# ictnlp/StreamSpeech

Measured on NVIDIA H100. Metric: audio-seconds/sec (RTF^-1) Fr-En simul S2ST @chunk=320ms, higher is better.
Workload: dtype f32

## Files before the change

### streamspeech_b200/csrc/engine.h

```cpp
#pragma once
#include <cuda_runtime.h>

#include <map>
#include <tuple>
#include <utility>
#include <string>
#include <vector>

#include "../../include/streamspeech_b200.h"
#include "kernels.h"
#include "kernels_persist.h"
#include "kernels_multistream.h"

namespace ss {

struct HostTensor {
  std::vector<float> data;
  std::vector<int64_t> shape;
  int64_t numel() const {
    int64_t n = 1;
    for (auto s : shape) n *= s;
    return n;
  }
};
// ... 53 lines not shown
};

}

struct ss_engine {
  int device = 0;
  ss_config cfg{};
  std::string err;
  bool finalized = false;
  int attn_chunk = 8, conv_chunk = 8;
  int umma_vocoder = 0;
  int umma_linear = 0;
  int unit_grouped = 1;
  int umma_min_rows = 128;
  int umma_min_channels = 16;
  ss::Umma2Cache* umma2_cache = nullptr;
  int vocoder_streams = 1;
  cudaStream_t aux_stream[2] = {nullptr, nullptr};
  cudaEvent_t fork_event = nullptr, join_event[2] = {nullptr, nullptr};
  int vocoder_graph = 0;
  int graph_pdl = 0;
  cudaStream_t capture_stream = nullptr;
  std::map<std::tuple<int, uintptr_t, int, int, int>, std::pair<cudaGraphExec_t, int>> voc_graphs;
  float* persist_ffn_scratch = nullptr;
  float* cl_blobs = nullptr;
  int cluster_cooperative = 1;
  long long cl_steps = 0;
  int persistent_encoder_cluster = 0;
  int persistent_ffn_fused = 1;
  int fbank_tma = 1;
  int persistent_encoder = 1;
  std::map<std::string, ss::HostTensor> host;
  std::vector<void*> dev_allocs;

  ss::Linear sub_conv[2];
  ss::Linear enc_linear;
  std::vector<ss::ConformerLayerW> enc;
  int Tpos = 0;
  ss::Linear ctc_head[2];
  ss::Linear ctc_pair;
  unsigned* ctc_ticket = nullptr;
  float* mt_emb = nullptr;
  float* mt_pos = nullptr;
  int mt_pos_rows = 0;
  std::vector<ss::DecLayerW> mt;
  ss::LNorm mt_ln;
// ... 86 lines not shown
```

### streamspeech_b200/csrc/engine_run.cu

```cuda
#include <algorithm>
#include <cmath>
#include <cstring>
#include <stdexcept>
#include <tuple>

#include "engine.h"

using namespace ss;

namespace {

inline cudaStream_t S(void* s) { return (cudaStream_t)s; }

int check_launch(ss_engine* h, const char* where) {
  cudaError_t e = cudaGetLastError();
  if (e != cudaSuccess) return h->fail(SS_ERR_CUDA, std::string(where) + ": " + cudaGetErrorString(e));
  return SS_OK;
}

thread_local int g_umma_linear = 0;
thread_local int g_umma_conv = 0;
thread_local int g_umma_min_rows = 128;
thread_local int g_umma_min_channels = 16;
thread_local Umma2Cache* g_umma2_cache = nullptr;
// ... 65 lines not shown
  Epilogue e;
  e.out = out; e.ldo = ldo; e.act = act;
  return e;
}
Epilogue ep_residual(float* inout, int ldo, float alpha = 1.0f) {
  Epilogue e;
  e.out = inout; e.ldo = ldo; e.alpha = alpha; e.residual = inout; e.res_scale = 1.0f;
  return e;
}

int report_async_error(ss_engine* h, unsigned flag, const char* where) {
  if (!flag) return SS_OK;
  cudaDeviceSynchronize();
  if (h->persist_bar) cudaMemset(h->persist_bar, 0, 64 * sizeof(unsigned));
  h->persist_bar_target = 0;
  return h->fail(SS_ERR_CUDA, std::string(where) + ": a grid barrier of a persistent kernel timed out; the results of the calls since the "
                                                   "last check are invalid (barrier re-armed)");
}

void clear_graphs(ss_engine* h) {
  cudaDeviceSynchronize();
  for (auto& kv : h->voc_graphs) cudaGraphExecDestroy(kv.second.first);
  h->voc_graphs.clear();
}

bool ws_begin(ss_engine* h, size_t bytes) {
  h->ws.reset();
  return h->ws.ensure(bytes);
}

struct DecScratch {
  float *y, *q, *kv, *attn, *hid, *qkv;
};

void dec_layer(const DecLayerW& L, float* x, int n, int dim, int ffn, int heads, bool causal, int self_kv_len_limit,
               const int* self_kv_len_dev, float* cache_k, float* cache_v, int past, const float* cross_kv, int Tk,
               const int* cross_len_dev, DecScratch& s, cudaStream_t st, int group_R = 0, const int* group_len_dev = nullptr) {
  const float scale = 0.125f;
  if (group_R > 1 && !cache_k && causal && n % group_R == 0) {
    const int S = n / group_R;
    ln_linear(x, dim * group_R, S, L.self_ln, L.qkv, ep_out(s.qkv, 3 * dim), s.y, st);
    grouped_causal_attention(s.qkv, 3 * dim, s.qkv + dim, 3 * dim, s.qkv + 2 * dim, 3 * dim, s.attn, dim, S, group_R, heads, scale, group_len_dev, st);
  } else if (cache_k) {
    ln_qkv_routed(x, dim, n, L.self_ln, L.qkv, dim, s.q, dim, cache_k + (size_t)past * dim, dim, cache_v + (size_t)past * dim, dim, s.y, st);
    mha_attention(s.q, dim, cache_k, dim, cache_v, dim, s.attn, dim, 1, n, past + n, heads, scale, 1, past, self_kv_len_dev, st);
  } else {
    ln_linear(x, dim, n, L.self_ln, L.qkv, ep_out(s.qkv, 3 * dim), s.y, st);
    mha_attention(s.qkv, 3 * dim, s.qkv + dim, 3 * dim, s.qkv + 2 * dim, 3 * dim, s.attn, dim, 1, n, n, heads, scale,
                  causal ? 1 : 0, 0, self_kv_len_dev, st);
  }
  (void)self_kv_len_limit;
// ... 774 lines not shown
  const int nrb = c.voc_n_rb;
  size_t total = ((size_t)N * c.voc_in_dim + (size_t)(2 + 4 * nrb) * maxbuf + (size_t)N * h->hop + 8192) * sizeof(float) + 64 * 256;
  if (!ws_begin(h, total)) return h->fail(SS_ERR_CUDA, "workspace allocation failed");
  float* frames = h->ws.f32((size_t)N * c.voc_in_dim);
  float* bufX = h->ws.f32(maxbuf);
  float* bufY = h->ws.f32(maxbuf);
  std::vector<float*> rbA(nrb), rbB(nrb), rbT(nrb), rbO(nrb);
  bool ok = frames && bufX && bufY;
  for (int j = 0; j < nrb; ++j) {
    rbA[j] = h->ws.f32(maxbuf); rbB[j] = h->ws.f32(maxbuf); rbT[j] = h->ws.f32(maxbuf); rbO[j] = h->ws.f32(maxbuf);
    ok = ok && rbA[j] && rbB[j] && rbT[j] && rbO[j];
  }
  float* wav = h->ws.f32((size_t)N * h->hop);
  if (!ok || !wav) return h->fail(SS_ERR_CUDA, "workspace too small");
  const bool fan_out = h->vocoder_streams && nrb == 3 && (g_umma_conv == 0 || g_umma_conv >= 12);
  if (fan_out && !h->fork_event) {
    bool made = cudaEventCreateWithFlags(&h->fork_event, cudaEventDisableTiming) == cudaSuccess;
    for (int i = 0; i < 2 && made; ++i)
      made = cudaStreamCreateWithFlags(&h->aux_stream[i], cudaStreamNonBlocking) == cudaSuccess &&
             cudaEventCreateWithFlags(&h->join_event[i], cudaEventDisableTiming) == cudaSuccess;
    if (!made) return h->fail(SS_ERR_CUDA, "cannot create the vocoder's auxiliary streams");
  }
  expand_frames(h->voc_unit_emb, h->voc_cumsum, h->voc_U, f_lo, N, c.voc_embedding_dim, frames, st);
  auto generator_body = [&](cudaStream_t st) {
  {
    ConvA a;
    a.x = frames; a.B = 1; a.L_in = N; a.L_rows = N; a.C_in = c.voc_in_dim; a.ldx = c.voc_in_dim; a.ksize = 7; a.pad_left = 3;
    Epilogue e = ep_out(bufX, c.voc_init_channels);
    e.bias = h->conv_pre.lin.b;
    conv_gemm(a, h->conv_pre.lin.w, c.voc_init_channels, e, st);
  }
  int L = N, ch = c.voc_init_channels;
  for (int i = 0; i < c.voc_n_ups; ++i) {
    const UpsampleW& U = h->ups[i];
    const int Lout = L * U.u;
    const bool fan_up = fan_out && U.u > 1;
    if (fan_up) {
      cudaEventRecord(h->fork_event, st);
      for (int q = 0; q < 2; ++q) cudaStreamWaitEvent(h->aux_stream[q], h->fork_event, 0);
    }
    for (int phi = 0; phi < U.u; ++phi) {
      int J = U.phase_J[phi], q0 = U.phase_q0[phi];
      int qmax = (Lout - 1 - phi + U.pad) / U.u;
      int nrows = qmax - q0 + 1;
      if (nrows <= 0) continue;
      const int lane = fan_up ? phi % 3 : 0;
// ... 111 lines not shown
  else if (n == "umma_linear") h->umma_linear = value;
  else if (n == "umma_min_rows") h->umma_min_rows = value;
  else if (n == "umma_min_channels") h->umma_min_channels = value;
  else if (n == "umma2_cache_clear") {
    umma2_cache_clear(h->umma2_cache);
    clear_graphs(h);
  }
  else if (n == "umma2_split_below") { g_umma2_split_below = value; clear_graphs(h); }
  else if (n == "umma2_min_units") { g_umma2_min_units = value; clear_graphs(h); }
  else if (n == "umma2_debug") {
    if (value && !g_umma2_dbg) {
      if (cudaMalloc(&g_umma2_dbg, 16 * sizeof(unsigned long long)) != cudaSuccess) return h->fail(SS_ERR_CUDA, "cudaMalloc failed");
      cudaMemset(g_umma2_dbg, 0, 16 * sizeof(unsigned long long));
    }
    if (!value && g_umma2_dbg) {
      cudaDeviceSynchronize();
      cudaFree(g_umma2_dbg);
      g_umma2_dbg = nullptr;
    }
  }
  else if (n == "prefer_shared") g_prefer_shared = value;
  else if (n == "unit_grouped") h->unit_grouped = value;
  else if (n == "vocoder_graph") h->vocoder_graph = value;
  else if (n == "graph_pdl") h->graph_pdl = value;
  else if (n == "fbank_tma") h->fbank_tma = value;
  else if (n == "umma2_fused_reduce") g_umma2_fused_reduce = value;
  else if (n == "persistent_encoder") h->persistent_encoder = value;
  else if (n == "persistent_ffn_fused") h->persistent_ffn_fused = value;
  else if (n == "cluster_cooperative") h->cluster_cooperative = value;
  else if (n == "persistent_encoder_cluster") {
    if (value && !h->cl_blobs) {
      if (!h->persist_layers || !h->persist_bar) return h->fail(SS_ERR_STATE, "persistent_encoder_cluster needs a finalized engine");
      const size_t n_f = encoder_layers_cluster_blob_floats(h->cfg.enc_layers);
      if (h->cfg.enc_dim != 256 || h->cfg.enc_ffn != 2048) return h->fail(SS_ERR_INVALID, "persistent_encoder_cluster: encoder must be 256 / 2048");
      if (cudaMalloc(&h->cl_blobs, n_f * sizeof(float)) != cudaSuccess) return h->fail(SS_ERR_CUDA, "cudaMalloc failed");
      h->dev_allocs.push_back(h->cl_blobs);
      encoder_layers_cluster_pack(h->persist_layers, h->cfg.enc_layers, h->cfg.dw_kernel, h->cl_blobs, 0);
      if (cudaDeviceSynchronize() != cudaSuccess) return h->fail(SS_ERR_CUDA, "packing the cluster weight blobs failed");
    }
    h->persistent_encoder_cluster = value;
  }
  else if (n == "vocoder_streams") h->vocoder_streams = value;
  else if (n == "persistent_mt") h->persistent_mt = value;
  else if (n == "persistent_mt_prefix") h->persistent_mt_prefix = value;
  else if (n == "persistent_mt_v2") h->persistent_mt_v2 = value;
  else if (n == "persistent_prefetch") h->persistent_prefetch = value;
// ... 142 lines not shown
```

### streamspeech_b200/csrc/kernels.h

```cpp
#pragma once
#include <cuda_runtime.h>
#include <stdint.h>

namespace ss {

extern unsigned long long g_launches;
extern int g_prefer_shared;
extern thread_local int g_pdl_off;

enum Act : int { ACT_NONE = 0, ACT_RELU = 1, ACT_SILU = 2, ACT_TANH = 3 };

struct ConvA {
  const float* x = nullptr;
  int B = 1;
  int L_in = 0;
  int L_rows = 0;
  int C_in = 0;
  int ldx = 0;
  int ksize = 1;
  int stride = 1;
  int dil = 1;
  int pad_left = 0;
  int chunk = 0;
  float pre_lrelu = 1.0f;
// ... 20 lines not shown
  const float* ln_beta = nullptr;
  int split_n = 0;
  float* out2 = nullptr;
  float* out3 = nullptr;
  int ldo2 = 0, ldo3 = 0;
};

void gemm_conv(const ConvA& a, const float* W, int N, const Epilogue& ep, cudaStream_t st);

float* splitk_workspace(size_t bytes);
unsigned* splitk_counters(int n_tiles);
void set_splitk_slot(int slot);
void splitk_epilogue(const float* ws, int splits, int M, int N, int L_rows, const Epilogue& ep, cudaStream_t st);

struct Umma2Cache;
extern int g_umma2_split_below, g_umma2_min_units;
extern int g_umma2_fused_reduce;
extern unsigned long long* g_umma2_dbg;
Umma2Cache* umma2_cache_create();
void umma2_cache_clear(Umma2Cache* c);
void umma2_cache_destroy(Umma2Cache* c);
bool umma2_supported(const ConvA& a, int N, const Epilogue& ep);
void umma2_conv(Umma2Cache* cache, const ConvA& a, const float* W, int N, const Epilogue& ep, int pieces, cudaStream_t st);

bool skinny_gemm_supported(int M, int N, int K, const Epilogue& ep);
void skinny_gemm(const float* A, int lda, const float* W, int M, int N, int K, const Epilogue& ep, cudaStream_t st);

void layer_norm(const float* x, int ldx, float* y, int ldy, const float* gamma, const float* beta, int rows, int C,
                cudaStream_t st);

void fbank_cmvn(const float* samples, int64_t n_samples, int f0, int nf, const float* mel_bank ,
                const float* window , const float* cmvn_mean, const float* cmvn_inv_std_or_null,
                const float* cmvn_std, float* out , cudaStream_t st);

void fbank_cmvn_tma(const float* samples, int f0, int nf, const float* melT, const float* window, const float* cmvn_mean, const float* cmvn_std,
                    float* out, cudaStream_t st);

void relpos_attention(const float* q, int ldq, const float* k, int ldk, const float* v, int ldv, const float* pos, int Tpos,
                      const float* bias_u, const float* bias_v, float* out, int B, int nQ, int q_offset, int T, int H, int D,
                      int chunk , const int* lengths_dev, cudaStream_t st);

void mha_attention(const float* q, int ldq, const float* k, int ldk, const float* v, int ldv, float* out, int ldo, int B,
                   int Tq, int Tk, int H, float scale, int causal, int causal_offset, const int* kv_len_dev,
                   cudaStream_t st);

void grouped_causal_attention(const float* q, int ldq, const float* k, int ldk, const float* v, int ldv, float* out, int ldo, int S, int R,
// ... 27 lines not shown
```

### streamspeech_b200/csrc/kernels_persist.cu

```cuda
#include <cooperative_groups.h>

#include "common.cuh"
#include "kernels.h"
#include "kernels_persist.h"

namespace cg = cooperative_groups;

namespace ss {
namespace {

constexpr int PW = 8;
constexpr int PT = PW * 32;
constexpr int PMR = 16;
constexpr int PHD = 64;
constexpr int PD = 256;

__device__ __forceinline__ unsigned long long globaltimer_ns() {
  unsigned long long t;
  asm volatile("mov.u64 %0, %globaltimer;" : "=l"(t));
  return t;
}

__device__ __forceinline__ float4 ldw(const float* p) {
  float4 r;
  asm volatile("ld.global.nc.L1::no_allocate.v4.f32 {%0, %1, %2, %3}, [%4];" : "=f"(r.x), "=f"(r.y), "=f"(r.z), "=f"(r.w) : "l"(p));
  return r;
}

__device__ __forceinline__ void grid_barrier(unsigned* ctr, unsigned& target) {
  __syncthreads();
  target += gridDim.x;
  if (threadIdx.x == 0) {
    asm volatile("red.release.gpu.global.add.u32 [%0], 1;" ::"l"(ctr) : "memory");
    unsigned v, spins = 0;
    do {
      asm volatile("ld.relaxed.gpu.global.u32 %0, [%1];" : "=r"(v) : "l"(ctr) : "memory");
    } while ((int)(v - target) < 0 && ++spins < (1u << 20));
    if ((int)(v - target) < 0) atomicExch(ctr + SS_BAR_ERR_WORD, 1u);
    asm volatile("fence.acq_rel.gpu;" ::: "memory");
  }
  __syncthreads();
}

__device__ __forceinline__ void prefetch_l2(const float* p, int n_floats) {
  const int lines = n_floats >> 5;
  for (int i = blockIdx.x * PT + threadIdx.x; i < lines; i += gridDim.x * PT)
    asm volatile("prefetch.global.L2 [%0];" ::"l"(p + (size_t)i * 32));
}

__device__ __forceinline__ void prefetch_layer(const PersistLayer& L, int D, int FFN) {
  prefetch_l2(L.ffn1_w1, D * FFN);
  prefetch_l2(L.ffn1_w2, D * FFN);
  prefetch_l2(L.wqkv, 3 * D * D);
  prefetch_l2(L.wo, D * D);
  prefetch_l2(L.pw1, 2 * D * D);
  prefetch_l2(L.pw2, D * D);
  prefetch_l2(L.ffn2_w1, D * FFN);
  prefetch_l2(L.ffn2_w2, D * FFN);
}

struct GemmEpi {
  const float* bias = nullptr;
  int act = ACT_NONE;
  float alpha = 1.f;
// ... 671 lines not shown
```

### streamspeech_b200/csrc/kernels_persist.h

```cpp
#pragma once
#include <cuda_runtime.h>
#include <stdint.h>

namespace ss {

#define SS_BAR_ERR_WORD 32

struct PersistLayer {
  const float *ffn1_g, *ffn1_b, *ffn1_w1, *ffn1_b1, *ffn1_w2, *ffn1_b2;
  const float *attn_g, *attn_b, *wqkv, *bqkv, *wo, *bo, *pos_u, *pos_v, *pos_proj;
  const float *conv_g, *conv_b, *pw1, *pw1_b, *dw_w, *bn_scale, *bn_shift, *pw2, *pw2_b;
  const float *ffn2_g, *ffn2_b, *ffn2_w1, *ffn2_b1, *ffn2_w2, *ffn2_b2;
  const float *fin_g, *fin_b;
  const float *ffn1_w2t, *ffn2_w2t;
};

bool encoder_layers_persistent_supported(int nA, int D, int FFN, int H, int T, int dw_k);
int encoder_layers_persistent(const PersistLayer* layers_dev, int n_layers, float* x, float* hid, float* qb, float* att, float* dw, float* kc,
                              float* vc, float* gc, int nA, int a0, int T, int D, int FFN, int H, int Tpos, int chunk, int conv_chunk, int dw_k,
                              unsigned long long* timestamps_or_null, unsigned* barrier_counter_dev_or_null,
                              unsigned* barrier_target_host, int prefetch ,
                              float* ffn_scratch_or_null , cudaStream_t st);

size_t encoder_layers_cluster_blob_floats(int n_layers);
void encoder_layers_cluster_pack(const PersistLayer* layers_dev, int n_layers, int dw_k, float* blobs_dev, cudaStream_t st);
bool encoder_layers_cluster_supported(int nA, int D, int FFN, int H, int T, int dw_k);
int encoder_layers_cluster(const PersistLayer* layers_dev, const float* blobs_dev, int n_layers, float* x, float* kc, float* vc, float* gc, int nA,
                           int a0, int T, int Tpos, int chunk, int conv_chunk, int dw_k, unsigned* bar_ctr, unsigned* bar_target_host,
                           unsigned long long* ts_or_null, const float* const* pos_proj_host , int cooperative ,
// ... 29 lines not shown
```

### streamspeech_b200/csrc/kernels_persist_mt.cu

```cuda
#include "common.cuh"
#include "kernels.h"
#include "kernels_persist.h"

namespace ss {
namespace {

constexpr int MW = 8;
constexpr int MTT = MW * 32;
constexpr int MHD = 64;

__device__ __forceinline__ float4 ldw(const float* p) {
  float4 r;
  asm volatile("ld.global.nc.L1::no_allocate.v4.f32 {%0, %1, %2, %3}, [%4];" : "=f"(r.x), "=f"(r.y), "=f"(r.z), "=f"(r.w) : "l"(p));
  return r;
}

__device__ __forceinline__ void grid_barrier(unsigned* ctr, unsigned& target) {
  __syncthreads();
  target += gridDim.x;
  if (threadIdx.x == 0) {
    asm volatile("red.release.gpu.global.add.u32 [%0], 1;" ::"l"(ctr) : "memory");
    unsigned v, spins = 0;
    do {
      asm volatile("ld.relaxed.gpu.global.u32 %0, [%1];" : "=r"(v) : "l"(ctr) : "memory");
    } while ((int)(v - target) < 0 && ++spins < (1u << 20));
    if ((int)(v - target) < 0) atomicExch(ctr + SS_BAR_ERR_WORD, 1u);
    asm volatile("fence.acq_rel.gpu;" ::: "memory");
  }
  __syncthreads();
}

struct MtSmem {
  float x[512];
  float v[2048];
  float S[1024];
  float qh[MHD];
  float pv[16][MHD];
  float red[MW];
  float rbest[MW];
  int ridx[MW];
  int tok;
};

__device__ __forceinline__ float block_reduce_sum(MtSmem& sm, float v) {
  const int lane = threadIdx.x & 31, w = threadIdx.x >> 5;
  v = warp_sum(v);
  __syncthreads();
  if (lane == 0) sm.red[w] = v;
  __syncthreads();
  float t = sm.red[0];
#pragma unroll
  for (int i = 1; i < MW; ++i) t += sm.red[i];
// ... 713 lines not shown
```

### streamspeech_b200/csrc/kernels_persist_mtp.cu

```cuda
#include "common.cuh"
#include "kernels.h"
#include "kernels_persist.h"

namespace ss {
namespace {

constexpr int QW = 8;
constexpr int QT = QW * 32;
constexpr int QRB = 16;
constexpr int QMAXM = 64;
constexpr int QD = 512;
constexpr int QFFN = 2048;
constexpr int QHD = 64;
constexpr int QMAXT = 1024;

__device__ __forceinline__ float4 ldw(const float* p) {
  float4 r;
  asm volatile("ld.global.nc.L1::no_allocate.v4.f32 {%0, %1, %2, %3}, [%4];" : "=f"(r.x), "=f"(r.y), "=f"(r.z), "=f"(r.w) : "l"(p));
  return r;
}

__device__ __forceinline__ void grid_barrier(unsigned* ctr, unsigned& target) {
  __syncthreads();
  target += gridDim.x;
  if (threadIdx.x == 0) {
    asm volatile("red.release.gpu.global.add.u32 [%0], 1;" ::"l"(ctr) : "memory");
    unsigned v, spins = 0;
    do {
      asm volatile("ld.relaxed.gpu.global.u32 %0, [%1];" : "=r"(v) : "l"(ctr) : "memory");
    } while ((int)(v - target) < 0 && ++spins < (1u << 20));
    if ((int)(v - target) < 0) atomicExch(ctr + SS_BAR_ERR_WORD, 1u);
    asm volatile("fence.acq_rel.gpu;" ::: "memory");
  }
  __syncthreads();
}

struct QSmem {
  float part[QW][4][QRB];
  float qs[QW][QHD];
};

__device__ __forceinline__ void stage_ln512(float* As, const float* x, int M, int Mpad, const float* __restrict__ g, const float* __restrict__ b,
                                            const int64_t* src_tok, const float* __restrict__ emb, const float* __restrict__ pos, int pad,
                                            float emb_scale, float* xg) {
  const int lane = threadIdx.x & 31, warp = threadIdx.x >> 5;
  float gv[16], bv[16];
#pragma unroll
  for (int i = 0; i < 16; ++i) {
    gv[i] = __ldg(g + lane + (i << 5));
    bv[i] = __ldg(b + lane + (i << 5));
  }
  for (int m0 = warp; m0 < Mpad; m0 += 2 * QW) {
    float v[2][16];
#pragma unroll
    for (int u = 0; u < 2; ++u) {
      const int m = m0 + u * QW;
      if (m < M) {
// ... 342 lines not shown
```

### streamspeech_b200/csrc/kernels_umma2.cu

```cuda
#include <cuda_bf16.h>

#include <algorithm>
#include <map>
#include <tuple>
#include <vector>

#include "common.cuh"
#include "kernels.h"

namespace ss {

struct Umma2Cache {
  std::map<std::tuple<const float*, int, int, int, int, int, int>, unsigned char*> packed;
  std::vector<void*> allocs;
};

namespace {

constexpr int U2_BM = 128;
constexpr int U2_CONVERTERS = 256;
constexpr int U2_THREADS = 288;
constexpr int U2_MAX_UNITS = 6;
constexpr int U2_MAX_SB = 4;
constexpr int U2_MAX_HALO = 64;

__device__ __forceinline__ uint32_t smem_u32(const void* p) { return (uint32_t)__cvta_generic_to_shared(p); }

__device__ __forceinline__ float u2_act(float x, int act) {
  switch (act) {
    case ACT_RELU: return x > 0.f ? x : 0.f;
    case ACT_SILU: return x / (1.0f + expf(-x));
// ... 454 lines not shown
  for (void* p : c->allocs) cudaFree(p);
  c->allocs.clear();
  c->packed.clear();
}

void umma2_cache_destroy(Umma2Cache* c) {
  if (!c) return;
  umma2_cache_clear(c);
  delete c;
}

bool umma2_supported(const ConvA& a, int N, const Epilogue& ep) {
  if (a.B != 1 || a.stride != 1 || a.chunk != 0 || a.lengths != nullptr) return false;
  if (a.t_offset != 0 || a.x_row0 != 0 || a.x_rows != 0) return false;
  if ((a.C_in & 15) != 0 || (a.ldx & 3) != 0 || a.C_in > a.ldx) return false;
  if ((reinterpret_cast<uintptr_t>(a.x) & 15) != 0) return false;
  if ((a.ksize - 1) * a.dil > U2_MAX_HALO || a.ksize < 1 || a.dil < 1) return false;
  if (N < 16 || (ep.glu && (N & 1))) return false;
  if (ep.ln_gamma != nullptr || ep.split_n > 0) return false;
  if (ep.out_L > 0 && a.L_rows <= 0) return false;
  return true;
}

void umma2_conv(Umma2Cache* cache, const ConvA& a, const float* W, int N, const Epilogue& ep, int pieces, cudaStream_t st) {
  ++g_launches;
  const int M = a.L_rows;
  if (M <= 0) return;
  const int NP = pieces >= 3 ? 3 : 2;
  const int BN = u2_bn(N);
  const int CK = (a.C_in % 32 == 0) ? 32 : 16;
  const int n_chunks = a.C_in / CK;
  const int n_tiles = (N + BN - 1) / BN;
  const int k = a.ksize;
  auto key = std::make_tuple(W, N, a.C_in, k, BN, NP, CK);
  unsigned char* wp = nullptr;
  auto it = cache->packed.find(key);
  if (it == cache->packed.end()) {
    const size_t bytes = (size_t)n_tiles * n_chunks * k * NP * BN * CK * 2;
    if (cudaMalloc((void**)&wp, bytes) != cudaSuccess) {
      cudaGetLastError();
      --g_launches;
      gemm_conv(a, W, N, ep, st);
      return;
    }
    cache->allocs.push_back(wp);
    cache->packed[key] = wp;
    const int64_t total = (int64_t)n_tiles * n_chunks * k * (CK >> 3) * BN;
    const int blocks = (int)((total + 255) / 256);
    if (NP == 3)
      umma2_pack_kernel<3><<<blocks, 256, 0, st>>>(W, N, a.C_in, k, BN, CK, n_tiles, wp);
    else
      umma2_pack_kernel<2><<<blocks, 256, 0, st>>>(W, N, a.C_in, k, BN, CK, n_tiles, wp);
  } else {
    wp = it->second;
  }
  U2Params p;
  p.a = a;
  p.ep = ep;
  p.wp = wp;
  p.M = M;
  p.N = N;
  p.CK = CK;
  p.ksize = k;
  p.dil = a.dil;
  p.rs = U2_BM + (k - 1) * a.dil;
  p.rs_pad = ((p.rs + 7) & ~7) + 4;
  p.units_total = n_chunks * k;
  const int m_tiles = (M + U2_BM - 1) / U2_BM;
  const long base = (long)m_tiles * n_tiles;
  const int min_units = std::max(1, g_umma2_min_units);
  int splits = 1;
  if (base < g_umma2_split_below && p.units_total >= 2 * min_units) {
    const long sms = std::max(1, current_device_sms());
    splits = (int)std::min<long>((sms + base - 1) / base, p.units_total / min_units);
    while (splits > 1 && (size_t)splits * M * N * sizeof(float) > (32u << 20)) --splits;
  }
  int ups = (p.units_total + splits - 1) / splits;
  splits = (p.units_total + ups - 1) / ups;
// ... 12 lines not shown
  const size_t a_bytes = (size_t)2 * NP * (CK >> 3) * p.rs_pad * 16;
  const size_t b_unit = (size_t)NP * BN * CK * 2;
  p.SB = (((a_bytes + 127) & ~(size_t)127) + 4 * b_unit <= 110 * 1024) ? 4 : 3;
  const size_t smem = std::max<size_t>(((a_bytes + 127) & ~(size_t)127) + p.SB * b_unit, (size_t)U2_BM * (BN + 8) * sizeof(float)) + 256;
  dim3 grid(n_tiles, m_tiles, splits);
  if (NP == 3) {
    switch (BN) {
      case 128: u2_launch<128, 3>(p, grid, smem, st); break;
      case 64: u2_launch<64, 3>(p, grid, smem, st); break;
      case 32: u2_launch<32, 3>(p, grid, smem, st); break;
      default: u2_launch<16, 3>(p, grid, smem, st); break;
    }
  } else {
    switch (BN) {
      case 128: u2_launch<128, 2>(p, grid, smem, st); break;
      case 64: u2_launch<64, 2>(p, grid, smem, st); break;
      case 32: u2_launch<32, 2>(p, grid, smem, st); break;
      default: u2_launch<16, 2>(p, grid, smem, st); break;
    }
  }
  if (splits > 1 && p.tile_ctr == nullptr) splitk_epilogue(ws, splits, M, N, a.L_rows, ep, st);
}

}
```

### streamspeech_b200/engine.py

```python
from __future__ import annotations

import ctypes
import os
from typing import Dict, List, Optional, Sequence, Tuple

import torch

from . import constants
from .config import ModelConfig

_HERE = os.path.dirname(os.path.abspath(__file__))
LIB_PATH = os.path.join(_HERE, "libstreamspeech_b200.so")
SS_MAX_UPS, SS_MAX_RB, SS_MAX_DIL = 8, 4, 4


class SSConfig(ctypes.Structure):
    _fields_ = (
        [(n, ctypes.c_int32) for n in (
            "feat_dim", "enc_dim", "enc_ffn", "enc_heads", "enc_layers", "dw_kernel", "conv_channels", "conv_kernel",
            "src_vocab", "tgt_vocab", "mt_dim", "mt_ffn", "mt_heads", "mt_layers",
            "t2u_layers", "unit_dim", "unit_ffn", "unit_heads", "unit_layers", "unit_vocab", "ctc_upsample_rate",
            "bos", "pad", "eos", "unk", "uni_encoder", "max_enc_frames", "max_mt_positions", "voc_n_ups")]
        + [("voc_up_rates", ctypes.c_int32 * SS_MAX_UPS), ("voc_up_kernels", ctypes.c_int32 * SS_MAX_UPS),
           ("voc_init_channels", ctypes.c_int32), ("voc_n_rb", ctypes.c_int32),
# ... 148 lines not shown
                self._load("__const__.gcmvn_mean", torch.as_tensor(gcmvn["mean"], dtype=torch.float32))
                self._load("__const__.gcmvn_std", torch.as_tensor(gcmvn["std"], dtype=torch.float32))
            self._check(self.lib.ss_finalize(self._h))
        except Exception:
            self.close()
            raise
        self.set_option("prefer_shared", int(os.environ.get("SS_PREFER_SHARED", "0")))
        self.set_option("umma_vocoder", int(os.environ.get("SS_UMMA_VOCODER", "12")))
        self.set_option("umma_linear", int(os.environ.get("SS_UMMA_LINEAR", "13")))
        self.set_option("umma_min_rows", int(os.environ.get("SS_UMMA_MIN_ROWS", "128")))
        self.set_option("umma_min_channels", int(os.environ.get("SS_UMMA_MIN_CHANNELS", "16")))
        self.set_option("persistent_encoder", int(os.environ.get("SS_PERSISTENT_ENCODER", "1")))
        self.set_option("persistent_mt", int(os.environ.get("SS_PERSISTENT_MT", "1")))
        self.set_option("umma2_fused_reduce", int(os.environ.get("SS_UMMA2_FUSED_REDUCE", "0")))
        self.set_option("fbank_tma", int(os.environ.get("SS_FBANK_TMA", "1")))
        self.set_option("persistent_ffn_fused", int(os.environ.get("SS_PERSISTENT_FFN_FUSED", "1")))
        self.set_option("persistent_encoder_cluster", int(os.environ.get("SS_PERSISTENT_ENCODER_CLUSTER", "1")))
        self.set_option("cluster_cooperative", int(os.environ.get("SS_CLUSTER_COOPERATIVE", "1")))
        self.set_option("persistent_mt_v2", int(os.environ.get("SS_PERSISTENT_MT_V2", "1")))
        self.set_option("persistent_mt_prefix", int(os.environ.get("SS_PERSISTENT_MT_PREFIX", "1")))
        self.set_option("vocoder_streams", int(os.environ.get("SS_VOCODER_STREAMS", "1")))
        self.set_option("unit_grouped", int(os.environ.get("SS_UNIT_GROUPED", "1")))
        self.set_option("vocoder_graph", int(os.environ.get("SS_VOCODER_GRAPH", "0")))
        self.set_option("graph_pdl", int(os.environ.get("SS_GRAPH_PDL", "0")))
        self.set_option("persistent_prefetch", int(os.environ.get("SS_PERSISTENT_PREFETCH", "0")))
        self.set_option("umma2_split_below", int(os.environ.get("SS_UMMA2_SPLIT_BELOW", "60")))
        self.set_option("umma2_min_units", int(os.environ.get("SS_UMMA2_MIN_UNITS", "4")))
        self.set_option("persistent_barrier", int(os.environ.get("SS_PERSISTENT_BARRIER", "1")))
        self.hop = self.lib.ss_vocoder_hop(self._h)
        self.vocoder_receptive_field = self.lib.ss_vocoder_receptive_field(self._h)

    def close(self):
        if getattr(self, "_h", None) is not None and self._h:
            self.lib.ss_destroy(self._h)
            self._h = None

    def __del__(self):
        try:
            self.close()
        except Exception:
            pass

    def _check(self, rc: int):
        if rc != 0:
            raise EngineError(f"libstreamspeech_b200 error {rc}: {self.lib.ss_last_error(self._h).decode()}")

# ... 284 lines not shown
```

Measured before the change: 125.8.

## Fuse the whole HiFi-GAN vocoder into one persistent cooperative wgmma kernel

Adds a persistent cooperative kernel that runs the whole vocoder (conv_pre, the upsample phases, the resblock convs and conv_post) as phases of work items separated by grid barriers. It uses wgmma tiles with packed weights and caches a job table per frame count and workspace base. The goal is to remove the many per-layer launches and the launch gaps in the vocoder for streaming-sized chunks. In exchange, phases must sync across the grid and the tile shapes are fixed. conv_post is a naive scalar loop, and the barrier helper and weight packing are refactored into shared code.

```diff
diff --git a/streamspeech_b200/csrc/engine.h b/streamspeech_b200/csrc/engine.h
--- a/streamspeech_b200/csrc/engine.h
+++ b/streamspeech_b200/csrc/engine.h
@@ -99,6 +99,8 @@
   int graph_pdl = 0;
   cudaStream_t capture_stream = nullptr;
   std::map<std::tuple<int, uintptr_t, int, int, int>, std::pair<cudaGraphExec_t, int>> voc_graphs;
+  int vocoder_fused = -1;
+  std::map<std::pair<int, uintptr_t>, ss::VocFusedParams> voc_fused;
   float* persist_ffn_scratch = nullptr;
   float* cl_blobs = nullptr;
   int cluster_cooperative = 1;
diff --git a/streamspeech_b200/csrc/engine_run.cu b/streamspeech_b200/csrc/engine_run.cu
--- a/streamspeech_b200/csrc/engine_run.cu
+++ b/streamspeech_b200/csrc/engine_run.cu
@@ -111,11 +111,113 @@
   cudaDeviceSynchronize();
   for (auto& kv : h->voc_graphs) cudaGraphExecDestroy(kv.second.first);
   h->voc_graphs.clear();
+  h->voc_fused.clear();
 }
 
 bool ws_begin(ss_engine* h, size_t bytes) {
   h->ws.reset();
   return h->ws.ensure(bytes);
+}
+
+constexpr int kVocFusedMaxFrames = 1024;
+
+VocFusedParams* vocoder_fused_table(ss_engine* h, int N, const float* frames, float* bufX, float* bufY, const std::vector<float*>& rbA,
+                                                    const std::vector<float*>& rbB, const std::vector<float*>& rbT, const std::vector<float*>& rbO,
+                                                    cudaStream_t st) {
+  const auto key = std::make_pair(N, (uintptr_t)h->ws.base);
+  auto it = h->voc_fused.find(key);
+  if (it != h->voc_fused.end()) return &it->second;
+  const ss_config& c = h->cfg;
+  const int grid = vocoder_fused_grid();
+  if (grid <= 0) return nullptr;
+  std::vector<VocJob> jobs;
+  std::vector<VocPhase> phases;
+  int a_stride = 0, b_stride = 0;
+  bool ok = true;
+  auto job = [&](const float* x0, const float* x1, const float* x2, int L_in, int M, int C_in, int k, int dil, int pad_left, float slope,
+                 const float* W, const float* bias, float* out, int Nout, int stride, int offset, const float* residual, float alpha, float res_scale) {
+    VocJob j{};
+    j.x0 = x0; j.x1 = x1; j.x2 = x2; j.L_in = L_in; j.M = M; j.C_in = C_in; j.ksize = k; j.dil = dil; j.pad_left = pad_left; j.slope = slope;
+    j.wp = reinterpret_cast<const unsigned char*>(W);
+    j.bias = bias; j.out = out; j.N = Nout; j.out_row_stride = stride; j.out_row_offset = offset; j.residual = residual; j.alpha = alpha;
+    j.res_scale = res_scale;
+    j.CK = (C_in % 32 == 0) ? 32 : 16;
+    j.m_tiles = (M + VOC_FUSED_BM - 1) / VOC_FUSED_BM;
+    if (C_in % 16 != 0 || Nout % 16 != 0 || k < 1 || (k - 1) * dil > 50 || bias == nullptr) ok = false;
+    jobs.push_back(j);
+  };
+  auto phase = [&](int first) {
+    const int n_jobs = (int)jobs.size() - first;
+    int items32 = 0;
+    for (int i = first; i < (int)jobs.size(); ++i) items32 += jobs[i].N % 32 == 0 ? jobs[i].m_tiles * (jobs[i].N / 32) : 0;
+    const bool bn32 = items32 >= grid;
+    VocPhase p{first, n_jobs, 0};
+    for (int i = first; i < (int)jobs.size(); ++i) {
+      VocJob& j = jobs[i];
+      j.BN = (bn32 && j.N % 32 == 0) ? 32 : 16;
+      j.n_tiles = j.N / j.BN;
+      j.wp = umma2_packed_weights(h->umma2_cache, reinterpret_cast<const float*>(j.wp), j.N, j.C_in, j.ksize, j.BN, j.CK, 2, st);
+      if (j.wp == nullptr) ok = false;
+      const int rs_pad = ((VOC_FUSED_BM + (j.ksize - 1) * j.dil + 7) & ~7) + 4;
+      a_stride = std::max(a_stride, 2 * (j.CK / 8) * rs_pad * 16);
+      b_stride = std::max(b_stride, j.ksize * 2 * j.BN * j.CK * 2);
+      p.n_items += j.m_tiles * j.n_tiles;
+    }
+    std::stable_sort(jobs.begin() + first, jobs.end(), [](const VocJob& a, const VocJob& b) { return a.ksize > b.ksize; });
+    phases.push_back(p);
+  };
+  jobs.reserve(1 + c.voc_n_ups * (8 + 2 * c.voc_n_rb * c.voc_rb_ndil));
+  job(frames, nullptr, nullptr, N, N, c.voc_in_dim, 7, 1, 3, 1.0f, h->conv_pre.lin.w, h->conv_pre.lin.b, bufX, c.voc_init_channels, 1, 0, nullptr,
+      1.0f, 1.0f);
+  phase(0);
+  const int nrb = c.voc_n_rb, nd = c.voc_rb_ndil;
+  int L = N;
+  for (int i = 0; i < c.voc_n_ups; ++i) {
+    const UpsampleW& U = h->ups[i];
+    const int Lout = L * U.u;
+    const float* x0 = i == 0 ? bufX : rbO[0];
+    const float* x1 = i == 0 ? nullptr : rbO[1];
+    const float* x2 = i == 0 ? nullptr : rbO[2];
+    int first = (int)jobs.size();
+    for (int phi = 0; phi < U.u; ++phi) {
+      const int J = U.phase_J[phi], q0 = U.phase_q0[phi];
+      const int nrows = (Lout - 1 - phi + U.pad) / U.u - q0 + 1;
+      if (nrows <= 0) continue;
+      job(x0, x1, x2, L, nrows, U.cin, J, 1, (J - 1) - q0, 0.1f, U.phase_w[phi].w, U.bias, bufY, U.cout, U.u, q0 * U.u + phi - U.pad, nullptr,
+          1.0f, 1.0f);
+    }
+    phase(first);
+    L = Lout;
+    const int ch = U.cout;
+    for (int m = 0; m < nd; ++m) {
+      first = (int)jobs.size();
+      for (int j = 0; j < nrb; ++j) {
+        const ConvW& w1 = h->rb1[i][j][m];
+        const float* cur = m == 0 ? bufY : (m == 1 ? rbA[j] : rbB[j]);
+        job(cur, nullptr, nullptr, L, L, ch, w1.ksize, w1.dil, (w1.ksize * w1.dil - w1.dil) / 2, 0.1f, w1.lin.w, w1.lin.b, rbT[j], ch, 1, 0,
+            nullptr, 1.0f, 1.0f);
+      }
+      phase(first);
+      first = (int)jobs.size();
+      for (int j = 0; j < nrb; ++j) {
+        const ConvW& w2 = h->rb2[i][j][m];
+        const float* cur = m == 0 ? bufY : (m == 1 ? rbA[j] : rbB[j]);
+        float* out = m + 1 < nd ? (m == 0 ? rbA[j] : rbB[j]) : rbO[j];
+        const float s = m + 1 < nd ? 1.0f : 1.0f / nrb;
+        job(rbT[j], nullptr, nullptr, L, L, ch, w2.ksize, 1, (w2.ksize - 1) / 2, 0.1f, w2.lin.w, w2.lin.b, out, ch, 1, 0, cur, s, s);
+      }
+      phase(first);
+    }
+  }
+  if (!ok || jobs.size() > VOC_MAX_JOBS || phases.size() > VOC_MAX_PHASES || vocoder_fused_smem(a_stride, b_stride) > 200 * 1024) return nullptr;
+  if (h->voc_fused.size() >= 64) h->voc_fused.clear();
+  VocFusedParams& p = h->voc_fused[key];
+  std::copy(jobs.begin(), jobs.end(), p.jobs);
+  std::copy(phases.begin(), phases.end(), p.phases);
+  p.n_phases = (int)phases.size();
+  p.a_stride = a_stride;
+  p.b_stride = b_stride;
+  return &p;
 }
 
 struct DecScratch {
@@ -936,6 +1038,19 @@
     if (!made) return h->fail(SS_ERR_CUDA, "cannot create the vocoder's auxiliary streams");
   }
   expand_frames(h->voc_unit_emb, h->voc_cumsum, h->voc_U, f_lo, N, c.voc_embedding_dim, frames, st);
+  const bool fused = h->vocoder_fused != 0 && (h->vocoder_fused == 1 || N <= kVocFusedMaxFrames) && g_umma_conv == 12 && nrb == 3 &&
+                     h->persist_bar != nullptr;
+  if (fused) {
+    VocFusedParams* P = vocoder_fused_table(h, N, frames, bufX, bufY, rbA, rbB, rbT, rbO, st);
+    if (P) {
+      VocPost& post = P->post;
+      post.x0 = rbO[0]; post.x1 = rbO[1]; post.x2 = rbO[2];
+      post.w = h->conv_post_w; post.bias = h->conv_post_b; post.slope = 0.01f;
+      post.L = N * h->hop; post.C = h->conv_post_c; post.k = h->conv_post_k; post.t0 = ctx * h->hop;
+      post.out = wav_out_dev;
+      if (vocoder_fused(*P, h->persist_bar, &h->persist_bar_target, st) == 0) return check_launch(h, "ss_vocoder_generate");
+    }
+  }
   auto generator_body = [&](cudaStream_t st) {
   {
     ConvA a;
@@ -1093,6 +1208,7 @@
   else if (n == "prefer_shared") g_prefer_shared = value;
   else if (n == "unit_grouped") h->unit_grouped = value;
   else if (n == "vocoder_graph") h->vocoder_graph = value;
+  else if (n == "vocoder_fused") h->vocoder_fused = value;
   else if (n == "graph_pdl") h->graph_pdl = value;
   else if (n == "fbank_tma") h->fbank_tma = value;
   else if (n == "umma2_fused_reduce") g_umma2_fused_reduce = value;
diff --git a/streamspeech_b200/csrc/kernels.h b/streamspeech_b200/csrc/kernels.h
--- a/streamspeech_b200/csrc/kernels.h
+++ b/streamspeech_b200/csrc/kernels.h
@@ -66,6 +66,42 @@
 void umma2_cache_destroy(Umma2Cache* c);
 bool umma2_supported(const ConvA& a, int N, const Epilogue& ep);
 void umma2_conv(Umma2Cache* cache, const ConvA& a, const float* W, int N, const Epilogue& ep, int pieces, cudaStream_t st);
+const unsigned char* umma2_packed_weights(Umma2Cache* cache, const float* W, int N, int C_in, int ksize, int BN, int CK, int NP, cudaStream_t st);
+
+struct VocJob {
+  const float *x0, *x1, *x2;
+  int L_in, M, C_in, ksize, dil, pad_left;
+  float slope;
+  const unsigned char* wp;
+  const float* bias;
+  float* out;
+  int N, out_row_stride, out_row_offset;
+  const float* residual;
+  float alpha, res_scale;
+  int BN, CK, m_tiles, n_tiles;
+};
+struct VocPhase {
+  int first_job, n_jobs, n_items;
+};
+struct VocPost {
+  const float *x0, *x1, *x2;
+  const float* w;
+  float bias, slope;
+  int L, C, k, t0;
+  float* out;
+};
+constexpr int VOC_FUSED_BM = 128;
+constexpr int VOC_MAX_JOBS = 128, VOC_MAX_PHASES = 48;
+struct VocFusedParams {
+  VocJob jobs[VOC_MAX_JOBS];
+  VocPhase phases[VOC_MAX_PHASES];
+  int n_phases;
+  int a_stride, b_stride;
+  VocPost post;
+};
+int vocoder_fused_grid();
+size_t vocoder_fused_smem(int a_stride, int b_stride);
+int vocoder_fused(const VocFusedParams& p, unsigned* bar_ctr, unsigned* bar_target_host, cudaStream_t st);
 
 bool skinny_gemm_supported(int M, int N, int K, const Epilogue& ep);
 void skinny_gemm(const float* A, int lda, const float* W, int M, int N, int K, const Epilogue& ep, cudaStream_t st);
diff --git a/streamspeech_b200/csrc/kernels_persist.cu b/streamspeech_b200/csrc/kernels_persist.cu
--- a/streamspeech_b200/csrc/kernels_persist.cu
+++ b/streamspeech_b200/csrc/kernels_persist.cu
@@ -25,21 +25,6 @@
   float4 r;
   asm volatile("ld.global.nc.L1::no_allocate.v4.f32 {%0, %1, %2, %3}, [%4];" : "=f"(r.x), "=f"(r.y), "=f"(r.z), "=f"(r.w) : "l"(p));
   return r;
-}
-
-__device__ __forceinline__ void grid_barrier(unsigned* ctr, unsigned& target) {
-  __syncthreads();
-  target += gridDim.x;
-  if (threadIdx.x == 0) {
-    asm volatile("red.release.gpu.global.add.u32 [%0], 1;" ::"l"(ctr) : "memory");
-    unsigned v, spins = 0;
-    do {
-      asm volatile("ld.relaxed.gpu.global.u32 %0, [%1];" : "=r"(v) : "l"(ctr) : "memory");
-    } while ((int)(v - target) < 0 && ++spins < (1u << 20));
-    if ((int)(v - target) < 0) atomicExch(ctr + SS_BAR_ERR_WORD, 1u);
-    asm volatile("fence.acq_rel.gpu;" ::: "memory");
-  }
-  __syncthreads();
 }
 
 __device__ __forceinline__ void prefetch_l2(const float* p, int n_floats) {
diff --git a/streamspeech_b200/csrc/kernels_persist.h b/streamspeech_b200/csrc/kernels_persist.h
--- a/streamspeech_b200/csrc/kernels_persist.h
+++ b/streamspeech_b200/csrc/kernels_persist.h
@@ -5,6 +5,23 @@
 namespace ss {
 
 #define SS_BAR_ERR_WORD 32
+
+#ifdef __CUDACC__
+__device__ __forceinline__ void grid_barrier(unsigned* ctr, unsigned& target) {
+  __syncthreads();
+  target += gridDim.x;
+  if (threadIdx.x == 0) {
+    asm volatile("red.release.gpu.global.add.u32 [%0], 1;" ::"l"(ctr) : "memory");
+    unsigned v, spins = 0;
+    do {
+      asm volatile("ld.relaxed.gpu.global.u32 %0, [%1];" : "=r"(v) : "l"(ctr) : "memory");
+    } while ((int)(v - target) < 0 && ++spins < (1u << 20));
+    if ((int)(v - target) < 0) atomicExch(ctr + SS_BAR_ERR_WORD, 1u);
+    asm volatile("fence.acq_rel.gpu;" ::: "memory");
+  }
+  __syncthreads();
+}
+#endif
 
 struct PersistLayer {
   const float *ffn1_g, *ffn1_b, *ffn1_w1, *ffn1_b1, *ffn1_w2, *ffn1_b2;
diff --git a/streamspeech_b200/csrc/kernels_persist_mt.cu b/streamspeech_b200/csrc/kernels_persist_mt.cu
--- a/streamspeech_b200/csrc/kernels_persist_mt.cu
+++ b/streamspeech_b200/csrc/kernels_persist_mt.cu
@@ -13,21 +13,6 @@
   float4 r;
   asm volatile("ld.global.nc.L1::no_allocate.v4.f32 {%0, %1, %2, %3}, [%4];" : "=f"(r.x), "=f"(r.y), "=f"(r.z), "=f"(r.w) : "l"(p));
   return r;
-}
-
-__device__ __forceinline__ void grid_barrier(unsigned* ctr, unsigned& target) {
-  __syncthreads();
-  target += gridDim.x;
-  if (threadIdx.x == 0) {
-    asm volatile("red.release.gpu.global.add.u32 [%0], 1;" ::"l"(ctr) : "memory");
-    unsigned v, spins = 0;
-    do {
-      asm volatile("ld.relaxed.gpu.global.u32 %0, [%1];" : "=r"(v) : "l"(ctr) : "memory");
-    } while ((int)(v - target) < 0 && ++spins < (1u << 20));
-    if ((int)(v - target) < 0) atomicExch(ctr + SS_BAR_ERR_WORD, 1u);
-    asm volatile("fence.acq_rel.gpu;" ::: "memory");
-  }
-  __syncthreads();
 }
 
 struct MtSmem {
diff --git a/streamspeech_b200/csrc/kernels_persist_mtp.cu b/streamspeech_b200/csrc/kernels_persist_mtp.cu
--- a/streamspeech_b200/csrc/kernels_persist_mtp.cu
+++ b/streamspeech_b200/csrc/kernels_persist_mtp.cu
@@ -18,21 +18,6 @@
   float4 r;
   asm volatile("ld.global.nc.L1::no_allocate.v4.f32 {%0, %1, %2, %3}, [%4];" : "=f"(r.x), "=f"(r.y), "=f"(r.z), "=f"(r.w) : "l"(p));
   return r;
-}
-
-__device__ __forceinline__ void grid_barrier(unsigned* ctr, unsigned& target) {
-  __syncthreads();
-  target += gridDim.x;
-  if (threadIdx.x == 0) {
-    asm volatile("red.release.gpu.global.add.u32 [%0], 1;" ::"l"(ctr) : "memory");
-    unsigned v, spins = 0;
-    do {
-      asm volatile("ld.relaxed.gpu.global.u32 %0, [%1];" : "=r"(v) : "l"(ctr) : "memory");
-    } while ((int)(v - target) < 0 && ++spins < (1u << 20));
-    if ((int)(v - target) < 0) atomicExch(ctr + SS_BAR_ERR_WORD, 1u);
-    asm volatile("fence.acq_rel.gpu;" ::: "memory");
-  }
-  __syncthreads();
 }
 
 struct QSmem {
diff --git a/streamspeech_b200/csrc/kernels_umma2.cu b/streamspeech_b200/csrc/kernels_umma2.cu
--- a/streamspeech_b200/csrc/kernels_umma2.cu
+++ b/streamspeech_b200/csrc/kernels_umma2.cu
@@ -7,6 +7,7 @@
 
 #include "common.cuh"
 #include "kernels.h"
+#include "kernels_persist.h"
 
 namespace ss {
 
@@ -507,38 +508,47 @@
   return true;
 }
 
+const unsigned char* umma2_packed_weights(Umma2Cache* cache, const float* W, int N, int C_in, int k, int BN, int CK, int NP, cudaStream_t st) {
+  auto key = std::make_tuple(W, N, C_in, k, BN, NP, CK);
+  auto it = cache->packed.find(key);
+  if (it != cache->packed.end()) return it->second;
+  const int n_chunks = C_in / CK;
+  const int n_tiles = (N + BN - 1) / BN;
+  unsigned char* wp = nullptr;
+  const size_t bytes = (size_t)n_tiles * n_chunks * k * NP * BN * CK * 2;
+  if (cudaMalloc((void**)&wp, bytes) != cudaSuccess) {
+    cudaGetLastError();
+    return nullptr;
+  }
+  cache->allocs.push_back(wp);
+  cache->packed[key] = wp;
+  const int64_t total = (int64_t)n_tiles * n_chunks * k * (CK >> 3) * BN;
+  const int blocks = (int)((total + 255) / 256);
+  if (NP == 3)
+    umma2_pack_kernel<3><<<blocks, 256, 0, st>>>(W, N, C_in, k, BN, CK, n_tiles, wp);
+  else
+    umma2_pack_kernel<2><<<blocks, 256, 0, st>>>(W, N, C_in, k, BN, CK, n_tiles, wp);
+  return wp;
+}
+
 void umma2_conv(Umma2Cache* cache, const ConvA& a, const float* W, int N, const Epilogue& ep, int pieces, cudaStream_t st) {
-  ++g_launches;
   const int M = a.L_rows;
-  if (M <= 0) return;
+  if (M <= 0) {
+    ++g_launches;
+    return;
+  }
   const int NP = pieces >= 3 ? 3 : 2;
   const int BN = u2_bn(N);
   const int CK = (a.C_in % 32 == 0) ? 32 : 16;
+  const int k = a.ksize;
+  const unsigned char* wp = umma2_packed_weights(cache, W, N, a.C_in, k, BN, CK, NP, st);
+  if (wp == nullptr) {
+    gemm_conv(a, W, N, ep, st);
+    return;
+  }
+  ++g_launches;
   const int n_chunks = a.C_in / CK;
   const int n_tiles = (N + BN - 1) / BN;
-  const int k = a.ksize;
-  auto key = std::make_tuple(W, N, a.C_in, k, BN, NP, CK);
-  unsigned char* wp = nullptr;
-  auto it = cache->packed.find(key);
-  if (it == cache->packed.end()) {
-    const size_t bytes = (size_t)n_tiles * n_chunks * k * NP * BN * CK * 2;
-    if (cudaMalloc((void**)&wp, bytes) != cudaSuccess) {
-      cudaGetLastError();
-      --g_launches;
-      gemm_conv(a, W, N, ep, st);
-      return;
-    }
-    cache->allocs.push_back(wp);
-    cache->packed[key] = wp;
-    const int64_t total = (int64_t)n_tiles * n_chunks * k * (CK >> 3) * BN;
-    const int blocks = (int)((total + 255) / 256);
-    if (NP == 3)
-      umma2_pack_kernel<3><<<blocks, 256, 0, st>>>(W, N, a.C_in, k, BN, CK, n_tiles, wp);
-    else
-      umma2_pack_kernel<2><<<blocks, 256, 0, st>>>(W, N, a.C_in, k, BN, CK, n_tiles, wp);
-  } else {
-    wp = it->second;
-  }
   U2Params p;
   p.a = a;
   p.ep = ep;
@@ -597,4 +607,219 @@
   if (splits > 1 && p.tile_ctr == nullptr) splitk_epilogue(ws, splits, M, N, a.L_rows, ep, st);
 }
 
-}
+namespace {
+
+constexpr int VF_THREADS = 256;
+constexpr int VF_UPT = 6;
+
+__device__ __forceinline__ void vf_cp_async16(uint32_t dst, const void* src) {
+  asm volatile("cp.async.cg.shared.global [%0], [%1], 16;" ::"r"(dst), "l"(src) : "memory");
+}
+
+template <int BN, bool ADD3>
+__device__ __forceinline__ void vf_item(const VocJob& J, int mt, int nt, unsigned char* a_smem, unsigned char* b_smem, float* tile,
+                                        uint32_t a_stride, uint32_t b_stride) {
+  constexpr int NACC = BN / 2;
+  constexpr int TP = BN + 8;
+  const int tid = threadIdx.x, warp = tid >> 5, lane = tid & 31, wg = warp >> 2;
+  const int m0 = mt * VOC_FUSED_BM, n0 = nt * BN;
+  const int CK = J.CK, k = J.ksize, dil = J.dil, C_in = J.C_in;
+  const int n_chunks = C_in / CK;
+  const int rs = VOC_FUSED_BM + (k - 1) * dil;
+  const uint32_t a_plane = (uint32_t)(((rs + 7) & ~7) + 4) * 16u;
+  const uint32_t a_piece = (uint32_t)(CK >> 3) * a_plane;
+  const uint32_t b_plane = (uint32_t)BN * 16u;
+  const uint32_t b_piece = (uint32_t)BN * CK * 2u;
+  const uint32_t b_unit = 2u * b_piece;
+  const uint32_t b_chunk = (uint32_t)k * b_unit;
+  const unsigned char* wsrc = J.wp + (size_t)nt * n_chunks * b_chunk;
+
+  const int upr_shift = (CK == 32) ? 3 : 2;
+  const int upr = 1 << upr_shift;
+  const int n_a = rs * upr;
+  int64_t goff[VF_UPT];
+  uint32_t soff[VF_UPT];
+#pragma unroll
+  for (int i = 0; i < VF_UPT; ++i) {
+    const int idx = tid + i * VF_THREADS;
+    const int r = idx >> upr_shift, q = idx & (upr - 1);
+    const int pos = m0 + r - J.pad_left;
+    const bool inb = idx < n_a && pos >= 0 && pos < J.L_in;
+    goff[i] = inb ? (int64_t)pos * C_in + q * 4 : (int64_t)-1;
+    soff[i] = (uint32_t)(q >> 1) * a_plane + (uint32_t)r * 16u + (uint32_t)(q & 1) * 8u;
+  }
+  float4 pf[ADD3 ? 3 : 1][VF_UPT];
+  auto load_a = [&](int c) {
+#pragma unroll
+    for (int i = 0; i < VF_UPT; ++i) {
+      const float4 z = make_float4(0.f, 0.f, 0.f, 0.f);
+      const int64_t o = goff[i] + (int64_t)c * CK;
+      pf[0][i] = goff[i] >= 0 ? __ldcg(reinterpret_cast<const float4*>(J.x0 + o)) : z;
+      if (ADD3) {
+        pf[ADD3 ? 1 : 0][i] = goff[i] >= 0 ? __ldcg(reinterpret_cast<const float4*>(J.x1 + o)) : z;
+        pf[ADD3 ? 2 : 0][i] = goff[i] >= 0 ? __ldcg(reinterpret_cast<const float4*>(J.x2 + o)) : z;
+      }
+    }
+  };
+  auto load_b = [&](int c, int s) {
+    const unsigned char* src = wsrc + (size_t)c * b_chunk;
+    const uint32_t dst = smem_u32(b_smem + (size_t)s * b_stride);
+    for (uint32_t i = tid; i < (b_chunk >> 4); i += VF_THREADS) vf_cp_async16(dst + 16u * i, src + 16u * i);
+    asm volatile("cp.async.commit_group;" ::: "memory");
+  };
+
+  float acc[NACC];
+#pragma unroll
+  for (int i = 0; i < NACC; ++i) acc[i] = 0.f;
+  load_b(0, 0);
+  load_a(0);
+  const float slope = J.slope;
+  for (int c = 0; c < n_chunks; ++c) {
+    const int s = c & 1;
+    unsigned char* stage = a_smem + (size_t)s * a_stride;
+#pragma unroll
+    for (int i = 0; i < VF_UPT; ++i) {
+      if (tid + i * VF_THREADS < n_a) {
+        float4 v = pf[0][i];
+        if (ADD3) {
+          const float4 b1 = pf[ADD3 ? 1 : 0][i], b2 = pf[ADD3 ? 2 : 0][i];
+          v = make_float4(b2.x + (b1.x + v.x), b2.y + (b1.y + v.y), b2.z + (b1.z + v.z), b2.w + (b1.w + v.w));
+        }
+        if (slope != 1.0f) {
+          v.x = v.x > 0.f ? v.x : v.x * slope;
+          v.y = v.y > 0.f ? v.y : v.y * slope;
+          v.z = v.z > 0.f ? v.z : v.z * slope;
+          v.w = v.w > 0.f ? v.w : v.w * slope;
+        }
+        u2_split_store<2>(v, stage, a_piece, soff[i]);
+      }
+    }
+    asm volatile("cp.async.wait_group 0;" ::: "memory");
+    asm volatile("fence.proxy.async.shared::cta;" ::: "memory");
+    __syncthreads();
+    if (c + 1 < n_chunks) {
+      load_b(c + 1, s ^ 1);
+      load_a(c + 1);
+    }
+    const uint32_t a_base = smem_u32(stage) + (uint32_t)wg * 64u * 16u;
+    const uint32_t b_base0 = smem_u32(b_smem + (size_t)s * b_stride);
+    u2_fence_acc<NACC>(acc);
+    asm volatile("wgmma.fence.sync.aligned;" ::: "memory");
+    for (int j = 0; j < k; ++j) {
+      const uint32_t a_tap = a_base + (uint32_t)(j * dil) * 16u;
+      const uint32_t b_base = b_base0 + (uint32_t)j * b_unit;
+      for (int ks = 0; ks < (CK >> 4); ++ks) {
+        const uint64_t a0 = u2_desc(a_tap + ks * 2 * a_plane, a_plane, 128), a1 = u2_desc(a_tap + a_piece + ks * 2 * a_plane, a_plane, 128);
+        const uint64_t b0 = u2_desc(b_base + ks * 2 * b_plane, b_plane, 128), b1 = u2_desc(b_base + b_piece + ks * 2 * b_plane, b_plane, 128);
+        u2_wgmma<BN>(acc, a0, b0);
+        u2_wgmma<BN>(acc, a0, b1);
+        u2_wgmma<BN>(acc, a1, b0);
+      }
+    }
+    asm volatile("wgmma.commit_group.sync.aligned;" ::: "memory");
+    asm volatile("wgmma.wait_group.sync.aligned 0;" ::: "memory");
+    u2_fence_acc<NACC>(acc);
+  }
+  {
+    const int r0 = wg * 64 + (warp & 3) * 16 + (lane >> 2);
+    const int c0 = 2 * (lane & 3);
+#pragma unroll
+    for (int i = 0; i < BN / 8; ++i) {
+      *reinterpret_cast<float2*>(tile + r0 * TP + 8 * i + c0) = make_float2(acc[4 * i], acc[4 * i + 1]);
+      *reinterpret_cast<float2*>(tile + (r0 + 8) * TP + 8 * i + c0) = make_float2(acc[4 * i + 2], acc[4 * i + 3]);
+    }
+  }
+  __syncthreads();
+  const int rows = min(VOC_FUSED_BM, J.M - m0);
+  for (int idx = tid; idx < rows * BN; idx += VF_THREADS) {
+    const int r = idx / BN, cc = idx - r * BN;
+    const int n = n0 + cc;
+    const int64_t o = ((int64_t)(m0 + r) * J.out_row_stride + J.out_row_offset) * J.N + n;
+    const float v = tile[r * TP + cc] + J.bias[n];
+    const float res = J.residual != nullptr ? J.res_scale * __ldcg(J.residual + o) : 0.f;
+    J.out[o] = J.alpha * v + res;
+  }
+  __syncthreads();
+}
+
+__global__ void __launch_bounds__(VF_THREADS, 1)
+    vocoder_fused_kernel(const __grid_constant__ VocFusedParams p, unsigned* bar_ctr, unsigned bar_target) {
+  extern __shared__ __align__(128) unsigned char smem[];
+  const uint32_t a_stride = (uint32_t)p.a_stride, b_stride = (uint32_t)p.b_stride;
+  unsigned char* a_smem = smem + ((128u - (smem_u32(smem) & 127u)) & 127u);
+  unsigned char* b_smem = a_smem + 2 * (size_t)a_stride;
+  float* tile = reinterpret_cast<float*>(b_smem + 2 * (size_t)b_stride);
+  const VocJob* jobs = p.jobs;
+  const VocPost& post = p.post;
+  for (int ph = 0; ph < p.n_phases; ++ph) {
+    const VocPhase P = p.phases[ph];
+    for (int i = blockIdx.x; i < P.n_items; i += gridDim.x) {
+      int jb = P.first_job, rest = i;
+      while (rest >= jobs[jb].m_tiles * jobs[jb].n_tiles) {
+        rest -= jobs[jb].m_tiles * jobs[jb].n_tiles;
+        ++jb;
+      }
+      const VocJob& J = jobs[jb];
+      const int nt = rest % J.n_tiles, mt = rest / J.n_tiles;
+      const bool add3 = J.x1 != nullptr;
+      if (J.BN == 32) {
+        if (add3) vf_item<32, true>(J, mt, nt, a_smem, b_smem, tile, a_stride, b_stride);
+        else vf_item<32, false>(J, mt, nt, a_smem, b_smem, tile, a_stride, b_stride);
+      } else {
+        if (add3) vf_item<16, true>(J, mt, nt, a_smem, b_smem, tile, a_stride, b_stride);
+        else vf_item<16, false>(J, mt, nt, a_smem, b_smem, tile, a_stride, b_stride);
+      }
+    }
+    grid_barrier(bar_ctr, bar_target);
+  }
+  const int half = (post.k - 1) >> 1;
+  for (int t = post.t0 + blockIdx.x * VF_THREADS + threadIdx.x; t < post.L; t += gridDim.x * VF_THREADS) {
+    float acc = post.bias;
+    for (int j = 0; j < post.k; ++j) {
+      const int p = t - half + j;
+      if (p < 0 || p >= post.L) continue;
+      const int64_t row = (int64_t)p * post.C;
+      for (int c = 0; c < post.C; ++c) {
+        float v = __ldcg(post.x2 + row + c) + (__ldcg(post.x1 + row + c) + __ldcg(post.x0 + row + c));
+        v = v > 0.f ? v : v * post.slope;
+        acc = fmaf(post.w[j * post.C + c], v, acc);
+      }
+    }
+    post.out[t - post.t0] = tanhf(acc);
+  }
+}
+
+}
+
+size_t vocoder_fused_smem(int a_stride, int b_stride) {
+  return 2 * (size_t)a_stride + 2 * (size_t)b_stride + (size_t)VOC_FUSED_BM * (32 + 8) * sizeof(float) + 128;
+}
+
+int vocoder_fused_grid() {
+  static const size_t smem_max = 200 * 1024;
+  if (first_time_on_device((const void*)vocoder_fused_kernel))
+    cudaFuncSetAttribute(vocoder_fused_kernel, cudaFuncAttributeMaxDynamicSharedMemorySize, (int)smem_max);
+  int occ = 0;
+  if (cudaOccupancyMaxActiveBlocksPerMultiprocessor(&occ, vocoder_fused_kernel, VF_THREADS, smem_max) != cudaSuccess) {
+    cudaGetLastError();
+    return 0;
+  }
+  return occ >= 1 ? current_device_sms() : 0;
+}
+
+int vocoder_fused(const VocFusedParams& p, unsigned* bar_ctr, unsigned* bar_target_host, cudaStream_t st) {
+  const int grid = vocoder_fused_grid();
+  const size_t smem = vocoder_fused_smem(p.a_stride, p.b_stride);
+  if (grid <= 0 || smem > 200 * 1024) return -1;
+  unsigned bar_target = *bar_target_host;
+  void* args[] = {(void*)&p, (void*)&bar_ctr, (void*)&bar_target};
+  if (cudaLaunchCooperativeKernel((void*)vocoder_fused_kernel, dim3(grid), dim3(VF_THREADS), args, smem, st) != cudaSuccess) {
+    cudaGetLastError();
+    return -2;
+  }
+  ++g_launches;
+  *bar_target_host += (unsigned)grid * (unsigned)p.n_phases;
+  return 0;
+}
+
+}
diff --git a/streamspeech_b200/engine.py b/streamspeech_b200/engine.py
--- a/streamspeech_b200/engine.py
+++ b/streamspeech_b200/engine.py
@@ -194,6 +194,7 @@
         self.set_option("vocoder_streams", int(os.environ.get("SS_VOCODER_STREAMS", "1")))
         self.set_option("unit_grouped", int(os.environ.get("SS_UNIT_GROUPED", "1")))
         self.set_option("vocoder_graph", int(os.environ.get("SS_VOCODER_GRAPH", "0")))
+        self.set_option("vocoder_fused", int(os.environ.get("SS_VOCODER_FUSED", "-1")))
         self.set_option("graph_pdl", int(os.environ.get("SS_GRAPH_PDL", "0")))
         self.set_option("persistent_prefetch", int(os.environ.get("SS_PERSISTENT_PREFETCH", "0")))
         self.set_option("umma2_split_below", int(os.environ.get("SS_UMMA2_SPLIT_BELOW", "60")))
```

After: 133.3 (median of 6 runs). 1.06x the previous value.
